# edouardlp/Mask-RCNN-CoreML

Measured on AMD Instinct MI355X. Metric: images/sec (1024x1024, COCO-80), higher is better.
Workload: dtype f32x3

## Files before the change

mask-rcnn-coreml_amd/_lib.py:

```python
from __future__ import annotations

import ctypes as C
import os

_HERE = os.path.dirname(os.path.abspath(__file__))
SO_PATH = os.environ.get("MRCNN_HIP_LIB") or os.path.join(_HERE, "libmaskrcnn_hip.so")

MRCNN_OK = 0
F32, F64, F16, U8, I32, F32S, F32X3 = 0, 1, 2, 3, 4, 5, 6
DEFAULT = -1
HOST, DEVICE = 0, 1
PARAM_INT, PARAM_DOUBLE, PARAM_STRING = 0, 1, 2
MODEL_MASKRCNN, MODEL_CLASSIFIER, MODEL_MASK = 0, 1, 2

EXPORTED_SYMBOLS = [
    "mrcnn_last_error", "mrcnn_version", "mrcnn_device_count", "mrcnn_config_set_anchors_path",
    "mrcnn_config_set_classifier_path", "mrcnn_config_set_mask_path", "mrcnn_config_get_anchors_path",
    "mrcnn_config_get_classifier_path", "mrcnn_config_get_mask_path", "mrcnn_layer_create",
    "mrcnn_layer_set_weight_data", "mrcnn_layer_output_shapes", "mrcnn_layer_evaluate", "mrcnn_layer_destroy",
    "mrcnn_iou", "mrcnn_model_load", "mrcnn_model_destroy", "mrcnn_model_set_stream", "mrcnn_maskrcnn_predict",
    "mrcnn_maskrcnn_predict_async", "mrcnn_maskrcnn_submit", "mrcnn_maskrcnn_collect", "mrcnn_classifier_predict", "mrcnn_mask_predict", "mrcnn_model_get_int",
    "mrcnn_model_read_tensor", "mrcnn_model_enable_timing", "mrcnn_model_stage_ms", "mrcnn_model_enable_graph",
    "mrcnn_detections_decode", "mrcnn_mask_to_u8", "mrcnn_paste_masks", "mrcnn_generate_anchors",
    "mrcnn_letterbox_geometry", "mrcnn_letterbox_rgb", "mrcnn_model_check_range", "mrcnn_model_calibrate_split", "mrcnn_model_split_group_stat",
# ... 10 lines not shown
    "mrcnn_jpeg_info", "mrcnn_jpeg_decode_host", "mrcnn_jpeg_decode_batch", "mrcnn_maskrcnn_predict_jpegs",
    "mrcnn_jpeg_decode_batch_on", "mrcnn_maskrcnn_predict_jpegs_on",
    "mrcnn_jpeg_encode_host", "mrcnn_jpeg_encode_batch",
    "mrcnn_png_encode_host", "mrcnn_png_encode_batch",
    "mrcnn_tile_plan", "mrcnn_maskrcnn_predict_tiles", "mrcnn_merge_tiles", "mrcnn_merge_tiles_host",
    "mrcnn_unite_tiles", "mrcnn_unite_tiles_host",
    "mrcnn_rle_decode", "mrcnn_rle_decode_host", "mrcnn_instance_map_rle", "mrcnn_instance_map_rle_host",
    "mrcnn_render_detections_rle", "mrcnn_render_detections_rle_host",
    "mrcnn_rle_to_polygons", "mrcnn_rle_to_polygons_host",
    "mrcnn_polygons_simplify", "mrcnn_polygons_simplify_host",
]
TEST_SYMBOLS = [
    "mrcnn_bench_conv", "mrcnn_bench_conv_dtype", "mrcnn_model_conv_profile_enable", "mrcnn_model_conv_profile_get",
    "mrcnn_model_conv_profile_shapes", "mrcnn_conv2d_nhwc", "mrcnn_debug_set", "mrcnn_bottleneck_nhwc", "mrcnn_bench_mfma_probe", "mrcnn_model_conv_profile_group", "mrcnn_bottleneck_first_nhwc", "mrcnn_bottleneck_stage_nhwc", "mrcnn_model_conv_profile_bytes",
    "mrcnn_jpeg_last_stage_ms", "mrcnn_jpeg_coefficients", "mrcnn_test_last_range_flag", "mrcnn_classifier_rows", "mrcnn_test_roi_align_nhwc_batch", "mrcnn_conv_chain_nhwc",
    "mrcnn_test_conv_form_nhwc",
]


class NativeLibraryMissing(RuntimeError):
    pass


class MrcnnError(RuntimeError):
    def __init__(self, code: int, msg: str):
        super().__init__(f"[mrcnn status {code}] {msg}")
        self.code = code


class Tensor(C.Structure):
    _fields_ = [("data", C.c_void_p), ("dtype", C.c_int32), ("memspace", C.c_int32),
# ... 169 lines not shown
    L.mrcnn_mask_to_u8.argtypes = [vp, C.c_int64, vp]
    L.mrcnn_mask_to_u8_f64.argtypes = [vp, C.c_int64, vp]
    ip = C.POINTER(C.c_int)
    L.mrcnn_letterbox_geometry.argtypes = [C.c_int] * 4 + [ip] * 4
    L.mrcnn_letterbox_rgb.argtypes = [vp, C.c_int, C.c_int, C.c_int, vp, C.c_int, C.c_int]
    L.mrcnn_generate_anchors.argtypes = [C.c_int, C.c_int, vp, C.c_int64, i64p]
    L.mrcnn_paste_masks.argtypes = [vp, C.c_int64, vp, C.c_int, C.c_int, C.c_int, C.c_int, C.c_float, C.c_int, vp]
    L.mrcnn_conv2d_nhwc.argtypes = [vp] + [C.c_int] * 4 + [vp] + [C.c_int] * 3 + [vp, vp, vp, C.c_int, C.c_int, vp]
    L.mrcnn_debug_set.argtypes = [cp, C.c_int]
    L.mrcnn_bench_mfma_probe.argtypes = [C.c_double, C.c_int, C.POINTER(C.c_double), C.POINTER(C.c_double)]
    L.mrcnn_bottleneck_first_nhwc.argtypes = [vp] + [C.c_int] * 4 + [vp] * 5 + [C.c_int, C.c_int, vp, vp]
    L.mrcnn_bottleneck_stage_nhwc.argtypes = [vp] + [C.c_int] * 4 + [vp] * 4 + [C.c_int, C.c_int, vp, vp, vp]
    L.mrcnn_bottleneck_nhwc.argtypes = [vp] + [C.c_int] * 4 + [vp] * 9 + [C.c_int, C.c_int, vp, vp]
    L.mrcnn_test_last_range_flag.argtypes = [ip]
    L.mrcnn_conv_chain_nhwc.argtypes = [vp] + [C.c_int] * 4 + [vp] * 5 + [C.c_int, C.c_int] + [vp] * 6 + [C.c_int] * 3 + [vp, vp]
    L.mrcnn_classifier_rows.argtypes = [vp, C.c_int64, vp, C.c_int, C.c_int64, vp, vp]
    L.mrcnn_model_check_range.argtypes = [vp, ip]
    L.mrcnn_model_calibrate_split.argtypes = [vp, vp, C.c_int, C.c_int, C.c_int, C.c_int, C.c_int]
    L.mrcnn_model_split_group_stat.argtypes = [vp, C.c_int, C.POINTER(SplitGroupStat)]
    L.mrcnn_model_get_split_exponents.argtypes = [vp, vp, C.c_int, ip]
    L.mrcnn_model_set_split_exponents.argtypes = [vp, vp, C.c_int]
    L.mrcnn_dist_rccl_shared.argtypes = []
    L.mrcnn_dist_rccl_shared.restype = C.c_int
    L.mrcnn_dist_unique_id.argtypes = [vp]
    L.mrcnn_dist_init.argtypes = [C.c_int, C.c_int, vp, C.POINTER(vp)]
    L.mrcnn_dist_destroy.argtypes = [vp]
    L.mrcnn_dist_destroy.restype = None
    L.mrcnn_dist_shard.argtypes = [C.c_int, C.c_int, C.c_int, ip, ip]
    L.mrcnn_dist_record_floats.argtypes = [C.c_int, C.c_int]
    L.mrcnn_dist_record_floats.restype = C.c_int64
# ... 39 lines not shown
```

mask-rcnn-coreml_amd/csrc/conv_dispatch.hip:

```cpp
#include "conv_device.h"
#include "knobs.h"

namespace mrcnn {

void conv_mfma_launch(hipStream_t s, const ConvArgs& a, int mode, int bn, bool wide_waves);
void conv_pp_launch(hipStream_t s, const ConvArgs& a, int mode);
void conv_chain_launch(hipStream_t s, const ConvArgs& p, const ConvArgs& q, int parts, bool wlds, int n_cus);

static inline int conv_wdtype(const ConvDesc& d) { return d.wdtype < 0 ? d.dtype : d.wdtype; }
static inline bool conv_is_split(const ConvDesc& d) { return d.dtype == MRCNN_F32 && (conv_wdtype(d) == MRCNN_F16 || conv_wdtype(d) == MRCNN_F32X3); }
static inline int conv_split_parts(const ConvDesc& d) { return conv_wdtype(d) == MRCNN_F32X3 ? 3 : 2; }
static inline bool conv_is_f16(const ConvDesc& d) { return d.dtype == MRCNN_F16 && (d.wdtype < 0 || d.wdtype == MRCNN_F16) && !d.out_f32; }
static inline bool is_pointwise(const ConvDesc& d) { return d.KH == 1 && d.KW == 1 && d.stride == 1 && !d.padH && !d.padW; }
static inline bool is_3x3_same(const ConvDesc& d) { return d.KH == 3 && d.KW == 3 && d.stride == 1 && d.padH == 1 && d.padW == 1; }
static inline bool dense_in(const ConvDesc& d, int h, int w, int c) { return d.H == h && d.W == w && d.Cin == c && d.in_sW == c && d.in_sH == (long)w * c && d.in_sB == (long)h * w * c; }
static inline bool dense_out(const ConvDesc& d, int h, int w, int c) { return d.OH == h && d.OW == w && d.Cout == c && d.out_sP == c && d.out_sB == (long)h * w * c; }
static inline bool plain_epilogue(const ConvDesc& d, int act) { return !d.out2 && !d.deconv2 && !d.sel_partial && !d.head_w && d.res_shift == 0 && d.act == act && d.scale && d.shift; }
static inline bool fills_chip(long tiles, int n_cus) { return tiles * 8 >= (long)n_cus * 7; }

static thread_local ConvProfile* g_prof = nullptr;
void conv_set_profiler(ConvProfile* p) { g_prof = p; }
static thread_local int* g_range_flag = nullptr;
void conv_set_range_flag(int* device_flag) { g_range_flag = device_flag; }
void ConvProfile::reset()
// ... 80 lines not shown
static int& g_tail = knob("conv_tail", "MRCNN_TAIL", 0);
static int& g_bneck = knob("conv_bneck", "MRCNN_BNECK", 1);
static int& g_bneck_stage = knob("conv_bneck_stage", "MRCNN_BNECK_STAGE", 0);
static int& g_c3h = knob("conv_c3h", "MRCNN_C3H", 1);
int conv_c3h_mode() { return g_c3h; }
bool conv_bneck_enabled() { return g_bneck != 0; }
static int& g_scfuse = knob("conv_scfuse", "MRCNN_SCFUSE", 1);
static int& g_sel_wave = knob("mask_sel_wave", "MRCNN_SEL_WAVE", 1);
int conv_sel_part_cols() { return g_sel_wave ? 64 : 128; }
static int& g_kchunk = knob("conv_kchunk", "MRCNN_KCHUNK", 1);
static int& g_ksplit = knob("conv_ksplit", "MRCNN_KSPLIT", 1);
static int& g_ksplit_below = knob("conv_ksplit_below", "MRCNN_KSPLIT_BELOW", 256);
static int& g_halo = knob("conv_halo", "MRCNN_HALO", 1);
bool conv_halo_enabled() { return g_halo != 0; }
static int& g_chain = knob("conv_chain", "MRCNN_CHAIN", 1);
static int& g_tn4 = knob("conv_tn4", nullptr, -1);

static int& g_pp = knob("conv_pp", "MRCNN_PP", 1);
static int& g_pp_min_tiles = knob("conv_pp_min_tiles", "MRCNN_PP_MIN_TILES", 512);
static int& g_pp_min_kt = knob("conv_pp_min_kt", "MRCNN_PP_MIN_KT", 16);
static int& g_pp_dbg = knob("conv_pp_dbg", "MRCNN_PP_DBG", 0);
static int& g_pp_min_fill = knob("conv_pp_min_fill", "MRCNN_PP_MIN_FILL", 85);
static int& g_pp_split = knob("conv_pp_split", "MRCNN_PP_SPLIT", 0);

static void conv_fill_args(const ConvDesc& d, ConvArgs& a)
{
    const bool half = d.dtype == MRCNN_F16;
    a.in = d.in; a.wgt = d.wgt; a.scale = d.scale; a.shift = d.shift; a.res = d.res; a.out = d.out; a.out2 = d.out2;
    a.in_sB = d.in_sB; a.in_sH = d.in_sH; a.in_sW = d.in_sW;
    a.res_sB = d.res_sB; a.res_sH = d.res_sH; a.res_sW = d.res_sW;
// ... 196 lines not shown
{
    if (!conv_is_split(d3) || !conv_is_split(d1) || conv_wdtype(d3) != conv_wdtype(d1)) return false;
    if (!d3.wgt_halo || !d1.wgt_halo || !conv_halo_eligible(d3) || d3.head_w || !conv_halo_tail_geometry_ok(d3.H, d3.W)) return false;
    if (d3.Npad != 256 || d3.act != ACT_RELU) return false;
    if (!conv_halo_tail_packable(d1.KH, d1.KW, d1.Cin, d1.Npad) || d1.Cout != 1024 || !is_pointwise(d1)) return false;
    if (d1.deconv2 || d1.out2 || d1.sel_partial || d1.act == ACT_SIGMOID || d1.res_shift || d1.head_w) return false;
    if (d1.in != d3.out || d1.B != d3.B || d1.OH != d3.OH || d1.OW != d3.OW) return false;
    if (!dense_out(d3, d3.OH, d3.OW, 256) || !dense_in(d1, d3.OH, d3.OW, 256)) return false;
    return true;
}

bool conv_chain_fusable(const ConvDesc& dP, const ConvDesc& dQ, const ConvDesc* sc)
{
    if (!conv_is_split(dP) || !conv_is_split(dQ) || conv_wdtype(dP) != conv_wdtype(dQ)) return false;
    const int C = dQ.Cout, H = dP.OH, W = dP.OW;
    if (!(C == 64 || C == 128) || dQ.Npad != C || dP.Cin != C || dP.Cout != 4 * C || dP.Npad != 4 * C) return false;
    if (!is_pointwise(dP) || !is_pointwise(dQ) || dP.B != dQ.B) return false;
    if (!plain_epilogue(dP, ACT_RELU) || !plain_epilogue(dQ, ACT_RELU) || dQ.res) return false;
    if (!dense_in(dP, H, W, C) || !dense_out(dP, H, W, 4 * C) || dQ.in != dP.out || !dense_in(dQ, H, W, 4 * C) || !dense_out(dQ, H, W, C)) return false;
    if (conv_k_chunks(dP) != 1 || conv_k_chunks(dQ) != 1) return false;
    auto al = [](const void* p) { return (reinterpret_cast<uintptr_t>(p) & 15) == 0; };
    if (!al(dP.in) || !al(dP.out) || !al(dQ.out) || !al(dP.wgt) || !al(dQ.wgt) || !al(dP.scale) || !al(dP.shift) || !al(dQ.scale) || !al(dQ.shift)) return false;
    if (sc) {
        if (!g_scfuse || !conv_shortcut_fusable(dP, *sc) || conv_k_chunks(*sc) != 1 || !sc->scale || !sc->shift) return false;
        if (C == 64 && sc->Cin != 64) return false;
        if (!al(sc->in) || !al(sc->wgt) || !al(sc->scale) || !al(sc->shift) || sc->in_sW % 4 || sc->in_sH % 4 || sc->in_sB % 4 || sc->Npad != 4 * C) return false;
    } else {
        if (!dP.res || !al(dP.res) || dP.res_sW != 4 * C || dP.res_sH != (long)W * 4 * C || dP.res_sB != (long)H * W * 4 * C) return false;
    }
    return true;
}

void conv_forward_chain(hipStream_t s, const ConvDesc& dP, const ConvDesc& dQ, const ConvDesc* sc)
{
    const long tiles = ((long)dP.B * dP.OH * dP.OW + 127) / 128;
    const bool sc_rides = g_chain >= 3 ? sc != nullptr && conv_chain_fusable(dP, dQ, sc) : conv_shortcut_rides(dP, sc);
    const int n_cus = device_cu_count();
    bool chain = g_chain && g_direct >= 2 && conv_chain_fusable(dP, dQ, sc_rides ? sc : nullptr) && (g_chain >= 2 || (dQ.Cout == 64 && fills_chip(tiles, n_cus)));
#ifndef MRCNN_CONV_ABLATE
    if (g_pp_dbg) chain = false;
#endif
    if (!chain) {
        conv_forward(s, dP, sc);
        conv_forward(s, dQ);
        return;
    }
    if (sc && !sc_rides) { conv_forward(s, *sc); sc = nullptr; }
    ConvDesc d = dP;
    if (sc) { d.res = nullptr; d.res_sB = d.res_sH = d.res_sW = 0; }
    ConvArgs aP, aQ;
    conv_fill_args(d, aP);
    conv_fill_args(dQ, aQ);
    if (sc) {
        aP.sc_in = sc->in; aP.sc_wgt = sc->wgt; aP.sc_scale = sc->scale; aP.sc_shift = sc->shift;
        aP.sc_in_sB = sc->in_sB; aP.sc_in_sH = sc->in_sH; aP.sc_in_sW = sc->in_sW;
        aP.sc_H = sc->H; aP.sc_W = sc->W; aP.sc_Cin = sc->Cin; aP.sc_stride = sc->stride;
    }
    const ProfScope prof(s);
    conv_chain_launch(s, aP, aQ, conv_split_parts(dP), dQ.Cout == 64, n_cus);
    if (prof) {
        const double fl = 2.0 * (double)aP.M * ((double)aP.ncols * (aP.Ktot + (sc ? sc->Cin : 0)) + (double)aQ.ncols * aQ.Ktot);
        prof.finish(sc ? TILE_128x128_4WAVE : TILE_128x128, fl, aP.M, aP.ncols, aP.Ktot, dP.group,
                    conv_algorithmic_bytes(d, sc) + conv_algorithmic_bytes(dQ) - (double)aP.M * dQ.Cin * 4.0);
    }
    HIP_CHECK(hipGetLastError());
}

void conv_forward_tail(hipStream_t s, const ConvDesc& d3, const ConvDesc& d1, const ConvDesc* sc, const ConvDesc* q)
{
    const int n_cus = device_cu_count();
    const long tiles = ((long)d3.B * d3.OH * d3.OW + 127) / 128;
    ConvArgs a3, a1;
    bool fuse = g_tail && g_halo && g_scratch && conv_tail_fusable(d3, d1) && fills_chip(tiles, n_cus);
    if (sc && fuse) { conv_forward(s, *sc); sc = nullptr; }
// ... 126 lines not shown
```

mask-rcnn-coreml_amd/csrc/conv_pack.h:

```cpp
#pragma once
#include <stddef.h>
#include <vector>

namespace mrcnn {

template <class Src>
std::vector<float> pack_filter_rows(int O, int I, int KH, int KW, int Npad, Src&& src)
{
    std::vector<float> w((size_t)Npad * KH * KW * I, 0.f);
    for (int o = 0; o < O; ++o)
        for (int y = 0; y < KH; ++y)
            for (int x = 0; x < KW; ++x)
                for (int i = 0; i < I; ++i) w[(((size_t)o * KH + y) * KW + x) * I + i] = src(o, y, x, i);
    return w;
}

inline int deconv2_row(int dy, int dx, int co, int O) { return (dy * 2 + dx) * O + co; }
template <class Src>
std::vector<float> pack_deconv2_rows(int I, int O, int Npad, Src&& src)
{
    std::vector<float> w((size_t)Npad * I, 0.f);
    for (int dy = 0; dy < 2; ++dy)
        for (int dx = 0; dx < 2; ++dx)
            for (int o = 0; o < O; ++o)
                for (int i = 0; i < I; ++i) w[(size_t)deconv2_row(dy, dx, o, O) * I + i] = src(dy, dx, o, i);
    return w;
}

}
```

mask-rcnn-coreml_amd/csrc/engine.h:

```cpp
#pragma once
#include <functional>
#include <map>
#include <mutex>
#include <memory>
#include <string>
#include <vector>

#include "kernels.h"

namespace mrcnn {

struct MrcwTensor {
    int dtype = 0;
    std::vector<uint32_t> dims;
    const unsigned char* data = nullptr;
    size_t nbytes = 0;
    size_t count() const { size_t n = 1; for (auto d : dims) n *= d; return n; }
};
struct MrcwFile {
    std::string path;
    std::vector<unsigned char> buf;
    std::map<std::string, int64_t> ints;
    std::map<std::string, double> doubles;
    std::map<std::string, std::string> strings;
// ... 4 lines not shown
    double get_double(const std::string& k, double dflt) const;
    std::string get_string(const std::string& k) const;
    const MrcwTensor& tensor(const std::string& name) const;
    std::vector<float> floats(const std::string& name) const;
};

inline int mode_act(int mode) { return (mode == MRCNN_F32S || mode == MRCNN_F32X3) ? MRCNN_F32 : mode; }
inline int mode_wgt(int mode) { return mode == MRCNN_F32 ? MRCNN_F32 : (mode == MRCNN_F32X3 ? MRCNN_F32X3 : MRCNN_F16); }

struct PackedConv {
    DevBuf wgt, scale, shift;
    std::vector<float> h_scale, h_shift;
    DevBuf wgt_halo;
    DevBuf wgt_c3h;
    DevBuf wgt_frag;
    int Cin = 0, Cout = 0, KH = 1, KW = 1, Npad = 0;
    int dtype = MRCNN_F32;
    int wdtype = MRCNN_F32;
};

struct Tensor4 {
    void* p = nullptr;
    int H = 0, W = 0, C = 0;
    long sB() const { return (long)H * W * C; }
};

using Op = std::function<void(hipStream_t, int )>;

struct SplitGroup {
    std::string name;
// ... 186 lines not shown
```

mask-rcnn-coreml_amd/csrc/engine_internal.h:

```cpp
#pragma once
#include "engine.h"

namespace mrcnn {

float half_to_float(uint16_t h);
void upload(DevBuf& d, const std::vector<float>& h);
PackedConv pack_conv_oihw(const MrcwFile& f, const std::string& conv, const std::string& bn, int mode);
PackedConv pack_conv1(const MrcwFile& f, int mode);
PackedConv pack_stacked_1x1(const MrcwFile& f, const std::vector<std::string>& names, int mode);
PackedConv pack_deconv2(const MrcwFile& f, const std::string& name, int mode);
void init_scaled_op(ScaledOp& op, const PackedConv* pc, int g_in, int g_out);

struct ConvView {
    void* p = nullptr;
    int H = 0, W = 0;
    long sB = 0, sH = 0, sW = 0;
};
inline ConvView dense_view(const void* p, int H, int W, int C)
{
    return {const_cast<void*>(p), H, W, (long)H * W * C, (long)W * C, (long)C};
}
inline ConvView view_of(const Tensor4& t) { return dense_view(t.p, t.H, t.W, t.C); }

enum : unsigned { RETILED_NONE = 0, RETILED_HALO = 1, RETILED_C3H = 2, RETILED_FRAG = 4, RETILED_ALL = 7 };

inline ConvDesc make_conv_desc(const PackedConv& pc, const float* scale, const float* shift, const ConvView& in, const ConvView& out,
                               int stride, int pad, int act, unsigned retiled)
{
    ConvDesc d;
    d.dtype = pc.dtype; d.wdtype = pc.wdtype;
    d.in = in.p; d.H = in.H; d.W = in.W; d.Cin = pc.Cin;
    d.in_sB = in.sB; d.in_sH = in.sH; d.in_sW = in.sW;
    d.wgt = pc.wgt.p; d.KH = pc.KH; d.KW = pc.KW; d.stride = stride; d.padH = d.padW = pad;
    if (retiled & RETILED_HALO) d.wgt_halo = pc.wgt_halo.p;
    if (retiled & RETILED_C3H) d.wgt_c3h = pc.wgt_c3h.p;
    if (retiled & RETILED_FRAG) d.wgt_frag = pc.wgt_frag.p;
    d.scale = scale; d.shift = shift;
    d.act = act;
    d.out = out.p; d.OH = out.H; d.OW = out.W; d.Cout = pc.Cout; d.Npad = pc.Npad;
    d.out_sB = out.sB; d.out_sP = out.sW;
    return d;
}
inline void set_residual(ConvDesc& d, const ConvView& res, int res_shift)
{
    d.res = res.p; d.res_sB = res.sB; d.res_sH = res.sH; d.res_sW = res.sW; d.res_shift = res_shift;
}

void run_conv_dense(hipStream_t s, const PackedConv& pc, const void* in, int B, int H, int W, void* out, int stride,
                    int pad, int act, const void* res = nullptr, int out_f32 = 0, const ScaledOp* sop = nullptr);

template <class F>
// ... 12 lines not shown
```

mask-rcnn-coreml_amd/csrc/engine_plan.hip:

```cpp
#include "engine_internal.h"

#include <math.h>
#include <string.h>

#include <fstream>

namespace mrcnn {

static void read_std(const MrcwFile& f, const std::string& prefix, float out[4])
{
    const float dflt[4] = {0.1f, 0.1f, 0.2f, 0.2f};
    const int64_t cnt = f.get_int(prefix + "bboxStdDev_count", 0);
    for (int i = 0; i < 4; ++i) out[i] = dflt[i];
    if (cnt == 4)
        for (int i = 0; i < 4; ++i) out[i] = (float)f.get_double(prefix + "bboxStdDev_" + std::to_string(i), dflt[i]);
}

void Model::load(int kind_, const std::string& path, int max_batch_, int dtype_)
{
    require_gpu();
    kind = kind_;
    max_batch = max_batch_ > 0 ? max_batch_ : 1;
    file.load(path);
    mode = dtype_;
// ... 299 lines not shown
        x = xo;
        g_x = g_c1;
    }

    void residual_stage(int st)
    {
        const int f1s[6] = {0, 0, 64, 128, 256, 512}, f3s[6] = {0, 0, 256, 512, 1024, 2048};
        Tensor4 stage_ta, stage_tb, stage_main, stage_alt;
        bool stage_fused = false, x_is_main = true;
        const int g_stage = m.new_split_group("C" + std::to_string(st));
        for (auto& b : blocks[st]) {
            const std::string p = std::to_string(st) + b;
            const bool first = b == "a";
            const int stride = (first && st > 2) ? 2 : 1;
            const int oh = x.H / stride, ow = x.W / stride;
            const bool chain_q = pending_tail.open && !first && (st == 2 || st == 3) && (m.mode == MRCNN_F32S || m.mode == MRCNN_F32X3);
            if (!chain_q) tail_flush();
            if (first) { stage_ta = T(oh, ow, f1s[st]); stage_tb = T(oh, ow, f1s[st]); }
            if (first && m.mode == MRCNN_F16 && blocks[st].size() > 1 && bneck_geometry_ok(f1s[st], oh, ow)) {
                stage_fused = true;
                stage_alt = T(oh, ow, f3s[st]);
            }
            const int g_a = m.new_split_group("res" + p + "_branch2a"), g_b = m.new_split_group("res" + p + "_branch2b");
            Tensor4 ta = stage_ta;
            Tensor4 tb = stage_tb;
            if (!first && stage_fused) {
                const Tensor4 to = x_is_main ? stage_alt : stage_main;
                bneck_op("res" + p + "_branch2a", "res" + p + "_branch2b", "res" + p + "_branch2c", x, ta, tb, to, g_x, g_a, g_b, g_stage);
                x = to;
                x_is_main = !x_is_main;
                g_x = g_stage;
// ... 200 lines not shown
```

mask-rcnn-coreml_amd/csrc/engine_weights.hip:

```cpp
#include "engine_internal.h"
#include "conv_pack.h"

#include <math.h>
#include <string.h>

#include <fstream>

namespace mrcnn {

float half_to_float(uint16_t h)
{
    const uint32_t sign = (uint32_t)(h & 0x8000u) << 16;
    uint32_t exp = (h >> 10) & 0x1Fu, man = h & 0x3FFu, f;
    if (exp == 0) {
        if (man == 0) f = sign;
        else {
            exp = 113;
            while ((man & 0x400u) == 0) { man <<= 1; --exp; }
            man &= 0x3FFu;
            f = sign | (exp << 23) | (man << 13);
        }
    } else if (exp == 31) f = sign | 0x7F800000u | (man << 13);
    else f = sign | ((exp + 112) << 23) | (man << 13);
    float r;
// ... 181 lines not shown
    MRCNN_REQUIRE(t.dims.size() == 4, MRCNN_ERR_IO, "%s/kernel is not 4-D", conv.c_str());
    const int O = t.dims[0], I = t.dims[1], KH = t.dims[2], KW = t.dims[3];
    const std::vector<float> k = f.floats(conv + "/kernel");
    PackedConv pc = new_pack(dtype, I, O, KH, KW);
    const std::vector<float> w = pack_filter_rows(O, I, KH, KW, pc.Npad, [&](int o, int y, int x, int i) { return k[(((size_t)o * I + i) * KH + y) * KW + x]; });
    std::vector<float> sc, sh;
    fold_bn(f, conv, bn, O, pc.Npad, sc, sh);
    finish_pack(pc, w, sc, sh);
    if (pc.wdtype != pc.dtype && conv_halo_packable(KH, KW, I, pc.Npad)) {
        conv_halo_pack(nullptr, pc.wgt.p, pc.Npad, I, pc.wgt_halo);
        HIP_CHECK(hipStreamSynchronize(nullptr));
    } else if (pc.wdtype != pc.dtype && conv_halo_tail_packable(KH, KW, I, pc.Npad) && O == pc.Npad) {
        conv_halo_pack(nullptr, pc.wgt.p, pc.Npad, I, pc.wgt_halo, 1);
        HIP_CHECK(hipStreamSynchronize(nullptr));
    }
    if (pc.dtype == MRCNN_F16 && pc.wdtype == MRCNN_F16 && conv3x3h_packable(KH, KW, I, O, pc.Npad)) {
        conv3x3h_pack(nullptr, pc.wgt.p, O, I, pc.wgt_c3h);
        HIP_CHECK(hipStreamSynchronize(nullptr));
    }
    if (pc.dtype == MRCNN_F16 && pc.wdtype == MRCNN_F16 && O == pc.Npad && bneck_frag_wanted(KH, KW, I, O)) {
        bneck_pack_frag(nullptr, pc.wgt.p, O, KH * KW * I, pc.wgt_frag);
        HIP_CHECK(hipStreamSynchronize(nullptr));
    }
    return pc;
}

PackedConv pack_conv1(const MrcwFile& f, int dtype)
{
    const MrcwTensor& t = f.tensor("conv1/kernel");
    MRCNN_REQUIRE(t.dims.size() == 4 && t.dims[1] == 3 && t.dims[2] == 7 && t.dims[3] == 7, MRCNN_ERR_IO, "conv1/kernel must be [O,3,7,7]");
// ... 68 lines not shown
```

mask-rcnn-coreml_amd/csrc/kernels.h:

```cpp
#pragma once
#include <stddef.h>
#include <algorithm>
#include <map>
#include <tuple>
#include <vector>

#include "common.h"

namespace mrcnn {


struct ProposalWorkspace {
    int B = 0, A = 0, K = 0, Kpad = 0, max_keep = 0, nblk = 0, W = 0;
    uint32_t* keys = nullptr;
    uint32_t* hist = nullptr;
    uint32_t* blockhist = nullptr;
    uint32_t* state = nullptr;
    uint64_t* cand = nullptr;
    int32_t* topk_idx = nullptr;
    float* boxes = nullptr;
    uint64_t* nms_mask = nullptr;
    int32_t* keep_idx = nullptr;
    int32_t* keep_count = nullptr;
    static size_t bytes(int B, int A, int K, int max_keep);
// ... 138 lines not shown
void png_encode_forward(hipStream_t s, const PngBuffers& b, int batch, long long total_blocks, int format, int rows);

enum Act { ACT_NONE = 0, ACT_RELU = 1, ACT_SIGMOID = 2 };

struct ConvDesc {
    int dtype = MRCNN_F32;
    int out_f32 = 0;
    int wdtype = -1;
    const void* in = nullptr;
    int B = 0, H = 0, W = 0, Cin = 0;
    long in_sB = 0, in_sH = 0, in_sW = 0;
    const void* wgt = nullptr;
    const void* wgt_halo = nullptr;
    const void* wgt_frag = nullptr;
    const void* wgt_c3h = nullptr;
    int prefer_c3h = 0;
    int KH = 1, KW = 1, stride = 1, padH = 0, padW = 0;
    const float* scale = nullptr;
    const float* shift = nullptr;
    const void* res = nullptr;
    long res_sB = 0, res_sH = 0, res_sW = 0;
    int res_shift = 0;
    int act = ACT_NONE;
    void* out = nullptr;
    int OH = 0, OW = 0, Cout = 0, Npad = 0;
    long out_sB = 0, out_sP = 0;
    void* out2 = nullptr;
    int n_split = 0;
    long out2_sB = 0, out2_sP = 0;
    int deconv2 = 0;
// ... 223 lines not shown
```

mask-rcnn-coreml_amd/csrc/kernels_conv_chain.hip:

```cpp
#include "conv_device.h"

namespace mrcnn {

struct ChainArgs { ConvArgs p, q; };

__device__ __forceinline__ void chain_stage_acc(float* stage, const f32x16& acc, int l31, int kk)
{
#pragma unroll
    for (int q = 0; q < 4; ++q)
        *reinterpret_cast<float4*>(&stage[l31 * 32 + (((2 * q + kk) ^ (l31 & 7)) << 2)]) = make_float4(acc[4 * q], acc[4 * q + 1], acc[4 * q + 2], acc[4 * q + 3]);
}

struct ChainParts { f16x8 hi, lo, lo2; };
template <int PARTS>
__device__ __forceinline__ ChainParts chain_split(const uint4 u0, const uint4 u1)
{
    ChainParts p;
    if constexpr (PARTS == 3) split_hi_mid_lo(u0, u1, p.hi, p.lo, p.lo2);
    else { split_hi_lo(u0, u1, p.hi, p.lo); p.lo2 = p.lo; }
    return p;
}
template <int PARTS, int N>
__device__ __forceinline__ void chain_mfma_parts(f32x16 (&acc)[N], const uint4 (&bv)[N], const ChainParts& pt)
{
    const f16x8 hi = pt.hi, lo = pt.lo, lo2 = pt.lo2;
    _Pragma("unroll") for (int j = 0; j < N; ++j) acc[j] = __builtin_amdgcn_mfma_f32_32x32x16_f16(__builtin_bit_cast(f16x8, bv[j]), hi, acc[j], 0, 0, 0);
    _Pragma("unroll") for (int j = 0; j < N; ++j) acc[j] = __builtin_amdgcn_mfma_f32_32x32x16_f16(__builtin_bit_cast(f16x8, bv[j]), lo, acc[j], 0, 0, 0);
    if constexpr (PARTS == 3)
        _Pragma("unroll") for (int j = 0; j < N; ++j) acc[j] = __builtin_amdgcn_mfma_f32_32x32x16_f16(__builtin_bit_cast(f16x8, bv[j]), lo2, acc[j], 0, 0, 0);
}

template <int C, int PARTS, bool SC, bool WLDS>
__global__ __launch_bounds__(WLDS ? 512 : 256, WLDS ? 1 : 2) void k_conv_chain(const ChainArgs ca)
{
    static_assert(!WLDS || C == 64, "the LDS-resident form holds C = 64's filters");
    constexpr int NW = WLDS ? 8 : 4, C4 = 4 * C, KT = C / 32, TNP = 2, TNQ = C / 32;
    constexpr int A_BYTES = WLDS ? 0 : KT * 32 * 128;
    constexpr int W_BYTES = WLDS ? C4 * C * 2 : 0;
    constexpr int WF_BYTES = W_BYTES * (SC ? 3 : 2);
    __shared__ __attribute__((aligned(16))) unsigned char smem[WF_BYTES + NW * (A_BYTES + 32 * 32 * 4)];
    const ConvArgs& a = ca.p;
    const ConvArgs& aq = ca.q;
    const int t = threadIdx.x;
    const int wave = t >> 6, lane = t & 63;
// ... 195 lines not shown
            float4 x = *reinterpret_cast<const float4*>(&stage[(8 * ps + rrow) * 32 + (((lane & 7) ^ rrow) << 2)]);
            x.x = x.x * sc.x + sh.x; x.y = x.y * sc.y + sh.y; x.z = x.z * sc.z + sh.z; x.w = x.w * sc.w + sh.w;
            if (reluq) { x.x = fmaxf(x.x, 0.f); x.y = fmaxf(x.y, 0.f); x.z = fmaxf(x.z, 0.f); x.w = fmaxf(x.w, 0.f); }
            if (ok[ps]) {
                out_of_range_q = out_of_range_q || !(fabsf(x.x) < 65504.0f) || !(fabsf(x.y) < 65504.0f) || !(fabsf(x.z) < 65504.0f) || !(fabsf(x.w) < 65504.0f);
                *reinterpret_cast<float4*>(outq + mrow[ps] * C + n) = x;
            }
        }
        __builtin_amdgcn_wave_barrier();
    }
    }
    if (a.range_flag && out_of_range) atomicOr(a.range_flag, 1);
    if (aq.range_flag && out_of_range_q) atomicOr(aq.range_flag, 1);
}

void conv_chain_launch(hipStream_t s, const ConvArgs& p, const ConvArgs& q, int parts, bool wlds, int n_cus)
{
    ChainArgs ca{p, q};
    dim3 grid((p.M + 127) / 128), block(256);
    const bool sc = p.sc_in != nullptr;
    const int C = q.Cout;
    MRCNN_REQUIRE((C == 64 || C == 128) && (parts == 2 || parts == 3), MRCNN_ERR_INVALID, "conv_chain_launch: C %d, %d parts", C, parts);
    if (wlds) {
        MRCNN_REQUIRE(C == 64 && (!sc || p.sc_Cin == 64) && n_cus > 0, MRCNN_ERR_INVALID, "conv_chain_launch: the LDS-resident form holds C = 64's filters");
        const int tiles256 = (p.M + 255) / 256;
        grid = dim3(tiles256 < n_cus ? tiles256 : n_cus); block = dim3(512);
#define MRCNN_CHAIN_W(P_, S_) hipLaunchKernelGGL((k_conv_chain<64, P_, S_, true>), grid, block, 0, s, ca)
        if (parts == 3) { if (sc) MRCNN_CHAIN_W(3, true); else MRCNN_CHAIN_W(3, false); }
        else { if (sc) MRCNN_CHAIN_W(2, true); else MRCNN_CHAIN_W(2, false); }
#undef MRCNN_CHAIN_W
        return;
    }
    MRCNN_REQUIRE(C == 128, MRCNN_ERR_INVALID, "conv_chain_launch: C = 64 runs the LDS-resident form");
#define MRCNN_CHAIN(C_, P_, S_) hipLaunchKernelGGL((k_conv_chain<C_, P_, S_, false>), grid, block, 0, s, ca)
    if (parts == 3) { if (sc) MRCNN_CHAIN(128, 3, true); else MRCNN_CHAIN(128, 3, false); }
    else { if (sc) MRCNN_CHAIN(128, 2, true); else MRCNN_CHAIN(128, 2, false); }
#undef MRCNN_CHAIN
// ... 4 lines not shown
```

Before: 457.0.

## Extend fused 1x1 conv chain to C=256 stage-4 pairs with LDS weight ring

Adds a new chain kernel for ResNet stage-4 identity blocks (C=256, 1024 expand). The expand conv's output is fed straight into the following reduce conv inside one kernel, so the intermediate activation is not written and re-read between launches. The fp16 filter chunks are prepacked into a swizzled stream image at load time and double-buffered into LDS with buffer_load ... lds DMA. This costs extra weight memory and one large-LDS block per CU, and it relies on hand-written inline asm and waitcnt counts.

```diff
diff --git a/mask-rcnn-coreml_amd/_lib.py b/mask-rcnn-coreml_amd/_lib.py
--- a/mask-rcnn-coreml_amd/_lib.py
+++ b/mask-rcnn-coreml_amd/_lib.py
@@ -48,7 +48,7 @@
     "mrcnn_bench_conv", "mrcnn_bench_conv_dtype", "mrcnn_model_conv_profile_enable", "mrcnn_model_conv_profile_get",
     "mrcnn_model_conv_profile_shapes", "mrcnn_conv2d_nhwc", "mrcnn_debug_set", "mrcnn_bottleneck_nhwc", "mrcnn_bench_mfma_probe", "mrcnn_model_conv_profile_group", "mrcnn_bottleneck_first_nhwc", "mrcnn_bottleneck_stage_nhwc", "mrcnn_model_conv_profile_bytes",
     "mrcnn_jpeg_last_stage_ms", "mrcnn_jpeg_coefficients", "mrcnn_test_last_range_flag", "mrcnn_classifier_rows", "mrcnn_test_roi_align_nhwc_batch", "mrcnn_conv_chain_nhwc",
-    "mrcnn_test_conv_form_nhwc",
+    "mrcnn_test_conv_form_nhwc", "mrcnn_test_chain_stream_image",
 ]
 
 
@@ -248,6 +248,7 @@
     L.mrcnn_bottleneck_nhwc.argtypes = [vp] + [C.c_int] * 4 + [vp] * 9 + [C.c_int, C.c_int, vp, vp]
     L.mrcnn_test_last_range_flag.argtypes = [ip]
     L.mrcnn_conv_chain_nhwc.argtypes = [vp] + [C.c_int] * 4 + [vp] * 5 + [C.c_int, C.c_int] + [vp] * 6 + [C.c_int] * 3 + [vp, vp]
+    L.mrcnn_test_chain_stream_image.argtypes = [vp, C.c_int, C.c_int, vp]
     L.mrcnn_classifier_rows.argtypes = [vp, C.c_int64, vp, C.c_int, C.c_int64, vp, vp]
     L.mrcnn_model_check_range.argtypes = [vp, ip]
     L.mrcnn_model_calibrate_split.argtypes = [vp, vp, C.c_int, C.c_int, C.c_int, C.c_int, C.c_int]
diff --git a/mask-rcnn-coreml_amd/csrc/conv_dispatch.hip b/mask-rcnn-coreml_amd/csrc/conv_dispatch.hip
--- a/mask-rcnn-coreml_amd/csrc/conv_dispatch.hip
+++ b/mask-rcnn-coreml_amd/csrc/conv_dispatch.hip
@@ -5,7 +5,7 @@
 
 void conv_mfma_launch(hipStream_t s, const ConvArgs& a, int mode, int bn, bool wide_waves);
 void conv_pp_launch(hipStream_t s, const ConvArgs& a, int mode);
-void conv_chain_launch(hipStream_t s, const ConvArgs& p, const ConvArgs& q, int parts, bool wlds, int n_cus);
+void conv_chain_launch(hipStream_t s, const ConvArgs& p, const ConvArgs& q, int parts, bool wlds, int n_cus, const void* p_stream, const void* q_stream);
 
 static inline int conv_wdtype(const ConvDesc& d) { return d.wdtype < 0 ? d.dtype : d.wdtype; }
 static inline bool conv_is_split(const ConvDesc& d) { return d.dtype == MRCNN_F32 && (conv_wdtype(d) == MRCNN_F16 || conv_wdtype(d) == MRCNN_F32X3); }
@@ -118,6 +118,7 @@
 static int& g_halo = knob("conv_halo", "MRCNN_HALO", 1);
 bool conv_halo_enabled() { return g_halo != 0; }
 static int& g_chain = knob("conv_chain", "MRCNN_CHAIN", 1);
+static int& g_chain4 = knob("conv_chain4", "MRCNN_CHAIN4", 1);
 static int& g_tn4 = knob("conv_tn4", nullptr, -1);
 
 static int& g_pp = knob("conv_pp", "MRCNN_PP", 1);
@@ -344,13 +345,14 @@
 {
     if (!conv_is_split(dP) || !conv_is_split(dQ) || conv_wdtype(dP) != conv_wdtype(dQ)) return false;
     const int C = dQ.Cout, H = dP.OH, W = dP.OW;
-    if (!(C == 64 || C == 128) || dQ.Npad != C || dP.Cin != C || dP.Cout != 4 * C || dP.Npad != 4 * C) return false;
+    if (!(C == 64 || C == 128 || C == 256) || dQ.Npad != C || dP.Cin != C || dP.Cout != 4 * C || dP.Npad != 4 * C) return false;
     if (!is_pointwise(dP) || !is_pointwise(dQ) || dP.B != dQ.B) return false;
     if (!plain_epilogue(dP, ACT_RELU) || !plain_epilogue(dQ, ACT_RELU) || dQ.res) return false;
     if (!dense_in(dP, H, W, C) || !dense_out(dP, H, W, 4 * C) || dQ.in != dP.out || !dense_in(dQ, H, W, 4 * C) || !dense_out(dQ, H, W, C)) return false;
     if (conv_k_chunks(dP) != 1 || conv_k_chunks(dQ) != 1) return false;
     auto al = [](const void* p) { return (reinterpret_cast<uintptr_t>(p) & 15) == 0; };
     if (!al(dP.in) || !al(dP.out) || !al(dQ.out) || !al(dP.wgt) || !al(dQ.wgt) || !al(dP.scale) || !al(dP.shift) || !al(dQ.scale) || !al(dQ.shift)) return false;
+    if (C == 256 && (sc || !dP.wgt_stream || !dQ.wgt_stream || !al(dP.wgt_stream) || !al(dQ.wgt_stream))) return false;
     if (sc) {
         if (!g_scfuse || !conv_shortcut_fusable(dP, *sc) || conv_k_chunks(*sc) != 1 || !sc->scale || !sc->shift) return false;
         if (C == 64 && sc->Cin != 64) return false;
@@ -366,7 +368,9 @@
     const long tiles = ((long)dP.B * dP.OH * dP.OW + 127) / 128;
     const bool sc_rides = g_chain >= 3 ? sc != nullptr && conv_chain_fusable(dP, dQ, sc) : conv_shortcut_rides(dP, sc);
     const int n_cus = device_cu_count();
-    bool chain = g_chain && g_direct >= 2 && conv_chain_fusable(dP, dQ, sc_rides ? sc : nullptr) && (g_chain >= 2 || (dQ.Cout == 64 && fills_chip(tiles, n_cus)));
+    const bool c4 = dQ.Cout == 256;
+    const int g = c4 ? g_chain4 : g_chain;
+    bool chain = g && g_direct >= 2 && !(c4 && sc) && conv_chain_fusable(dP, dQ, sc_rides ? sc : nullptr) && (g >= 2 || ((c4 || dQ.Cout == 64) && fills_chip(tiles, n_cus)));
 #ifndef MRCNN_CONV_ABLATE
     if (g_pp_dbg) chain = false;
 #endif
@@ -387,7 +391,7 @@
         aP.sc_H = sc->H; aP.sc_W = sc->W; aP.sc_Cin = sc->Cin; aP.sc_stride = sc->stride;
     }
     const ProfScope prof(s);
-    conv_chain_launch(s, aP, aQ, conv_split_parts(dP), dQ.Cout == 64, n_cus);
+    conv_chain_launch(s, aP, aQ, conv_split_parts(dP), dQ.Cout == 64, n_cus, dP.wgt_stream, dQ.wgt_stream);
     if (prof) {
         const double fl = 2.0 * (double)aP.M * ((double)aP.ncols * (aP.Ktot + (sc ? sc->Cin : 0)) + (double)aQ.ncols * aQ.Ktot);
         prof.finish(sc ? TILE_128x128_4WAVE : TILE_128x128, fl, aP.M, aP.ncols, aP.Ktot, dP.group,
diff --git a/mask-rcnn-coreml_amd/csrc/conv_pack.h b/mask-rcnn-coreml_amd/csrc/conv_pack.h
--- a/mask-rcnn-coreml_amd/csrc/conv_pack.h
+++ b/mask-rcnn-coreml_amd/csrc/conv_pack.h
@@ -27,4 +27,25 @@
     return w;
 }
 
+inline bool chain_stream_wanted(int KH, int KW, int I, int O) { return KH == 1 && KW == 1 && ((I == 256 && O == 1024) || (I == 1024 && O == 256)); }
+inline size_t chain_stream_pos_p(int C, int n, int k)
+{
+    const int r = n & 63;
+    return (size_t)(n >> 6) * 64 * C + ((size_t)(k >> 5) * 64 + r) * 32 + ((((k >> 3) & 3) ^ ((r >> 2) & 3)) << 3) + (k & 7);
 }
+inline size_t chain_stream_pos_q(int C, int n, int k)
+{
+    return (size_t)(k >> 6) * 64 * C + ((size_t)((k >> 5) & 1) * C + n) * 32 + ((((k >> 3) & 3) ^ ((n >> 2) & 3)) << 3) + (k & 7);
+}
+template <class T>
+std::vector<T> pack_chain_stream(const T* w, int C, bool q)
+{
+    static_assert(sizeof(T) == 2, "fp16 filters");
+    const int rows = q ? C : 4 * C, K = q ? 4 * C : C;
+    std::vector<T> img((size_t)rows * K);
+    for (int n = 0; n < rows; ++n)
+        for (int k = 0; k < K; ++k) img[q ? chain_stream_pos_q(C, n, k) : chain_stream_pos_p(C, n, k)] = w[(size_t)n * K + k];
+    return img;
+}
+
+}
diff --git a/mask-rcnn-coreml_amd/csrc/engine.h b/mask-rcnn-coreml_amd/csrc/engine.h
--- a/mask-rcnn-coreml_amd/csrc/engine.h
+++ b/mask-rcnn-coreml_amd/csrc/engine.h
@@ -42,6 +42,7 @@
     DevBuf wgt_halo;
     DevBuf wgt_c3h;
     DevBuf wgt_frag;
+    DevBuf wgt_stream;
     int Cin = 0, Cout = 0, KH = 1, KW = 1, Npad = 0;
     int dtype = MRCNN_F32;
     int wdtype = MRCNN_F32;
diff --git a/mask-rcnn-coreml_amd/csrc/engine_internal.h b/mask-rcnn-coreml_amd/csrc/engine_internal.h
--- a/mask-rcnn-coreml_amd/csrc/engine_internal.h
+++ b/mask-rcnn-coreml_amd/csrc/engine_internal.h
@@ -22,7 +22,7 @@
 }
 inline ConvView view_of(const Tensor4& t) { return dense_view(t.p, t.H, t.W, t.C); }
 
-enum : unsigned { RETILED_NONE = 0, RETILED_HALO = 1, RETILED_C3H = 2, RETILED_FRAG = 4, RETILED_ALL = 7 };
+enum : unsigned { RETILED_NONE = 0, RETILED_HALO = 1, RETILED_C3H = 2, RETILED_FRAG = 4, RETILED_STREAM = 8, RETILED_ALL = 15 };
 
 inline ConvDesc make_conv_desc(const PackedConv& pc, const float* scale, const float* shift, const ConvView& in, const ConvView& out,
                                int stride, int pad, int act, unsigned retiled)
@@ -35,6 +35,7 @@
     if (retiled & RETILED_HALO) d.wgt_halo = pc.wgt_halo.p;
     if (retiled & RETILED_C3H) d.wgt_c3h = pc.wgt_c3h.p;
     if (retiled & RETILED_FRAG) d.wgt_frag = pc.wgt_frag.p;
+    if (retiled & RETILED_STREAM) d.wgt_stream = pc.wgt_stream.p;
     d.scale = scale; d.shift = shift;
     d.act = act;
     d.out = out.p; d.OH = out.H; d.OW = out.W; d.Cout = pc.Cout; d.Npad = pc.Npad;
diff --git a/mask-rcnn-coreml_amd/csrc/engine_plan.hip b/mask-rcnn-coreml_amd/csrc/engine_plan.hip
--- a/mask-rcnn-coreml_amd/csrc/engine_plan.hip
+++ b/mask-rcnn-coreml_amd/csrc/engine_plan.hip
@@ -337,7 +337,7 @@
             const bool first = b == "a";
             const int stride = (first && st > 2) ? 2 : 1;
             const int oh = x.H / stride, ow = x.W / stride;
-            const bool chain_q = pending_tail.open && !first && (st == 2 || st == 3) && (m.mode == MRCNN_F32S || m.mode == MRCNN_F32X3);
+            const bool chain_q = pending_tail.open && !first && (st == 2 || st == 3 || (st == 4 && !pending_tail.has_sc)) && (m.mode == MRCNN_F32S || m.mode == MRCNN_F32X3);
             if (!chain_q) tail_flush();
             if (first) { stage_ta = T(oh, ow, f1s[st]); stage_tb = T(oh, ow, f1s[st]); }
             if (first && m.mode == MRCNN_F16 && blocks[st].size() > 1 && bneck_geometry_ok(f1s[st], oh, ow)) {
diff --git a/mask-rcnn-coreml_amd/csrc/engine_weights.hip b/mask-rcnn-coreml_amd/csrc/engine_weights.hip
--- a/mask-rcnn-coreml_amd/csrc/engine_weights.hip
+++ b/mask-rcnn-coreml_amd/csrc/engine_weights.hip
@@ -219,6 +219,13 @@
         conv_halo_pack(nullptr, pc.wgt.p, pc.Npad, I, pc.wgt_halo, 1);
         HIP_CHECK(hipStreamSynchronize(nullptr));
     }
+    if (pc.wdtype != pc.dtype && pc.dtype == MRCNN_F32 && O == pc.Npad && chain_stream_wanted(KH, KW, I, O) && conv.find("_branch2") != std::string::npos) {
+        std::vector<uint16_t> hw(w.size());
+        for (size_t i = 0; i < w.size(); ++i) hw[i] = float_to_half(w[i]);
+        const std::vector<uint16_t> img = pack_chain_stream(hw.data(), 256, I == 1024);
+        pc.wgt_stream.alloc(img.size() * 2);
+        HIP_CHECK(hipMemcpy(pc.wgt_stream.p, img.data(), img.size() * 2, hipMemcpyHostToDevice));
+    }
     if (pc.dtype == MRCNN_F16 && pc.wdtype == MRCNN_F16 && conv3x3h_packable(KH, KW, I, O, pc.Npad)) {
         conv3x3h_pack(nullptr, pc.wgt.p, O, I, pc.wgt_c3h);
         HIP_CHECK(hipStreamSynchronize(nullptr));
diff --git a/mask-rcnn-coreml_amd/csrc/kernels.h b/mask-rcnn-coreml_amd/csrc/kernels.h
--- a/mask-rcnn-coreml_amd/csrc/kernels.h
+++ b/mask-rcnn-coreml_amd/csrc/kernels.h
@@ -176,6 +176,7 @@
     const void* wgt_halo = nullptr;
     const void* wgt_frag = nullptr;
     const void* wgt_c3h = nullptr;
+    const void* wgt_stream = nullptr;
     int prefer_c3h = 0;
     int KH = 1, KW = 1, stride = 1, padH = 0, padW = 0;
     const float* scale = nullptr;
diff --git a/mask-rcnn-coreml_amd/csrc/kernels_conv_chain.hip b/mask-rcnn-coreml_amd/csrc/kernels_conv_chain.hip
--- a/mask-rcnn-coreml_amd/csrc/kernels_conv_chain.hip
+++ b/mask-rcnn-coreml_amd/csrc/kernels_conv_chain.hip
@@ -2,7 +2,7 @@
 
 namespace mrcnn {
 
-struct ChainArgs { ConvArgs p, q; };
+struct ChainArgs { ConvArgs p, q; const void *p_stream, *q_stream; };
 
 __device__ __forceinline__ void chain_stage_acc(float* stage, const f32x16& acc, int l31, int kk)
 {
@@ -20,14 +20,14 @@
     else { split_hi_lo(u0, u1, p.hi, p.lo); p.lo2 = p.lo; }
     return p;
 }
-template <int PARTS, int N>
-__device__ __forceinline__ void chain_mfma_parts(f32x16 (&acc)[N], const uint4 (&bv)[N], const ChainParts& pt)
+template <int PARTS, int N, int NA = N, int OFF = 0>
+__device__ __forceinline__ void chain_mfma_parts(f32x16 (&acc)[NA], const uint4 (&bv)[N], const ChainParts& pt)
 {
     const f16x8 hi = pt.hi, lo = pt.lo, lo2 = pt.lo2;
-    _Pragma("unroll") for (int j = 0; j < N; ++j) acc[j] = __builtin_amdgcn_mfma_f32_32x32x16_f16(__builtin_bit_cast(f16x8, bv[j]), hi, acc[j], 0, 0, 0);
-    _Pragma("unroll") for (int j = 0; j < N; ++j) acc[j] = __builtin_amdgcn_mfma_f32_32x32x16_f16(__builtin_bit_cast(f16x8, bv[j]), lo, acc[j], 0, 0, 0);
+    _Pragma("unroll") for (int j = 0; j < N; ++j) acc[OFF + j] = __builtin_amdgcn_mfma_f32_32x32x16_f16(__builtin_bit_cast(f16x8, bv[j]), hi, acc[OFF + j], 0, 0, 0);
+    _Pragma("unroll") for (int j = 0; j < N; ++j) acc[OFF + j] = __builtin_amdgcn_mfma_f32_32x32x16_f16(__builtin_bit_cast(f16x8, bv[j]), lo, acc[OFF + j], 0, 0, 0);
     if constexpr (PARTS == 3)
-        _Pragma("unroll") for (int j = 0; j < N; ++j) acc[j] = __builtin_amdgcn_mfma_f32_32x32x16_f16(__builtin_bit_cast(f16x8, bv[j]), lo2, acc[j], 0, 0, 0);
+        _Pragma("unroll") for (int j = 0; j < N; ++j) acc[OFF + j] = __builtin_amdgcn_mfma_f32_32x32x16_f16(__builtin_bit_cast(f16x8, bv[j]), lo2, acc[OFF + j], 0, 0, 0);
 }
 
 template <int C, int PARTS, bool SC, bool WLDS>
@@ -253,13 +253,224 @@
     if (aq.range_flag && out_of_range_q) atomicOr(aq.range_flag, 1);
 }
 
-void conv_chain_launch(hipStream_t s, const ConvArgs& p, const ConvArgs& q, int parts, bool wlds, int n_cus)
-{
-    ChainArgs ca{p, q};
+template <int C, int PARTS>
+__global__ __launch_bounds__(256, 1) void k_conv_chain_ring(const ChainArgs ca)
+{
+    static_assert(C == 256, "the ring's stage holds C = 256's chunk images");
+    constexpr int C4 = 4 * C, KT = C / 32, TNP = 2, TNQ = C / 32, NCH = C4 / 64;
+    constexpr int WCH = 64 * C * 2;
+    constexpr int STAGE = 2 * WCH;
+    constexpr int NDMA = WCH / 4096;
+    __shared__ __attribute__((aligned(16))) unsigned char smem[2 * STAGE + 4 * 32 * 32 * 4];
+    __shared__ __attribute__((aligned(16))) float s_tab[2 * C4], s_tabq[2 * C];
+    const ConvArgs& a = ca.p;
+    const ConvArgs& aq = ca.q;
+    const int t = threadIdx.x;
+    const int wave = t >> 6, lane = t & 63;
+    const int l31 = lane & 31, kk = lane >> 5;
+    float* const stage = reinterpret_cast<float*>(smem + 2 * STAGE) + wave * (32 * 32);
+    static_assert(C4 == 4 * 256 && C % 8 == 0 && C / 2 <= 256, "the tables are filled by 256 threads, 16 B each");
+    *reinterpret_cast<float4*>(&s_tab[4 * t]) = *reinterpret_cast<const float4*>(a.scale + 4 * t);
+    *reinterpret_cast<float4*>(&s_tab[C4 + 4 * t]) = *reinterpret_cast<const float4*>(a.shift + 4 * t);
+    if (t < C / 2) *reinterpret_cast<float4*>(&s_tabq[4 * t]) = *reinterpret_cast<const float4*>(t < C / 4 ? aq.scale + 4 * t : aq.shift + 4 * (t - C / 4));
+    const float* const in = static_cast<const float*>(a.in);
+    const float* const res = static_cast<const float*>(a.res);
+    float* const out = static_cast<float*>(a.out);
+    float* const outq = static_cast<float*>(aq.out);
+    const int swzb = (l31 >> 2) & 3;
+
+    typedef unsigned srd_t __attribute__((ext_vector_type(4)));
+    srd_t srdP, srdQ;
+    {
+        const unsigned long long wp = (unsigned long long)(uintptr_t)ca.p_stream, wq = (unsigned long long)(uintptr_t)ca.q_stream;
+        srdP[0] = __builtin_amdgcn_readfirstlane((unsigned)wp);
+        srdP[1] = __builtin_amdgcn_readfirstlane((unsigned)(wp >> 32) & 0xffffu);
+        srdP[2] = (unsigned)(NCH * WCH);
+        srdP[3] = 0x00020000u;
+        srdQ[0] = __builtin_amdgcn_readfirstlane((unsigned)wq);
+        srdQ[1] = __builtin_amdgcn_readfirstlane((unsigned)(wq >> 32) & 0xffffu);
+        srdQ[2] = (unsigned)(NCH * WCH);
+        srdQ[3] = 0x00020000u;
+    }
+    const unsigned lds0 = __builtin_amdgcn_readfirstlane((unsigned)(uintptr_t)(__attribute__((address_space(3))) unsigned char*)smem);
+    const unsigned wdst = lds0 + (unsigned)__builtin_amdgcn_readfirstlane(wave) * 1024u;
+    const unsigned voff = (unsigned)t * 16u;
+#define MRCNN_RING_DMA(SRD, SOFF, DST)                                                                         \
+    asm volatile("s_nop 4\n\ts_mov_b32 m0, %3\n\ts_nop 0\n\tbuffer_load_dwordx4 %0, %1, %2 offen lds" ::"v"(voff), "s"(SRD), "s"(SOFF), "s"(DST) : "memory", "m0");
+    auto ring_fill = [&](int ch) {
+        const unsigned src = (unsigned)__builtin_amdgcn_readfirstlane(ch) * (unsigned)WCH;
+        const unsigned dst = wdst + (unsigned)(__builtin_amdgcn_readfirstlane(ch) & 1) * (unsigned)STAGE;
+#pragma unroll
+        for (int k = 0; k < NDMA; ++k) {
+            MRCNN_RING_DMA(srdP, src + k * 4096u, dst + k * 4096u)
+            MRCNN_RING_DMA(srdQ, src + k * 4096u, dst + (unsigned)WCH + k * 4096u)
+        }
+    };
+    ring_fill(0);
+
+    const int row0 = (blockIdx.x * 4 + __builtin_amdgcn_readfirstlane(wave)) * 32;
+    const bool live = row0 < a.M;
+    bool out_of_range = false, out_of_range_q = false;
+    ChainParts ap[2 * KT];
+    if (live) {
+        const int m = row0 + l31;
+        const bool m_ok = m < a.M;
+        const float* const src = in + (long)(m_ok ? m : row0) * C + 8 * kk;
+        uint4 u[2 * KT][2];
+#pragma unroll
+        for (int g = 0; g < 2 * KT; ++g) { u[g][0] = *reinterpret_cast<const uint4*>(src + g * 16); u[g][1] = *reinterpret_cast<const uint4*>(src + g * 16 + 4); }
+#pragma unroll
+        for (int g = 0; g < 2 * KT; ++g) {
+            if (!m_ok) u[g][0] = u[g][1] = make_uint4(0u, 0u, 0u, 0u);
+            ap[g] = chain_split<PARTS>(u[g][0], u[g][1]);
+        }
+    }
+    const bool full = row0 + 32 <= a.M;
+    const int rrow = lane >> 3, c4 = (lane & 7) * 4;
+    const bool relu = a.act == ACT_RELU, reluq = aq.act == ACT_RELU;
+    bool ok[4];
+    long mrow[4];
+#pragma unroll
+    for (int ps = 0; ps < 4; ++ps) { const int m = row0 + 8 * ps + rrow; ok[ps] = m < a.M; mrow[ps] = m; }
+
+    f32x16 accQ[TNQ];
+#pragma unroll
+    for (int j = 0; j < TNQ; ++j)
+#pragma unroll
+        for (int e = 0; e < 16; ++e) accQ[j][e] = 0.0f;
+
+    for (int ch = 0; ch < NCH; ++ch) {
+        if (full) asm volatile("s_waitcnt vmcnt(4)" ::: "memory");
+        else asm volatile("s_waitcnt vmcnt(0)" ::: "memory");
+        __syncthreads();
+        if (ch + 1 < NCH) ring_fill(ch + 1);
+        if (!live) continue;
+        const unsigned char* const w3s = smem + (ch & 1) * STAGE;
+        const unsigned char* const w1s = w3s + WCH;
+        const int nc = ch * 64;
+        float4 rv[TNP][4];
+#pragma unroll
+        for (int j = 0; j < TNP; ++j)
+#pragma unroll
+            for (int ps = 0; ps < 4; ++ps) {
+                rv[j][ps] = make_float4(0.f, 0.f, 0.f, 0.f);
+                if (res && ok[ps]) rv[j][ps] = *reinterpret_cast<const float4*>(res + mrow[ps] * C4 + nc + j * 32 + c4);
+            }
+        f32x16 accP[TNP];
+#pragma unroll
+        for (int j = 0; j < TNP; ++j)
+#pragma unroll
+            for (int e = 0; e < 16; ++e) accP[j][e] = 0.0f;
+        auto frag_p = [&](uint4 (&b)[TNP], int i) {
+#pragma unroll
+            for (int j = 0; j < TNP; ++j) b[j] = *reinterpret_cast<const uint4*>(w3s + ((i >> 1) * 64 + j * 32 + l31) * 64 + (((2 * (i & 1) + kk) ^ swzb) << 4));
+        };
+        {
+            uint4 bv[TNP];
+            frag_p(bv, 0);
+#pragma unroll
+            for (int i = 0; i < 2 * KT; ++i) {
+                uint4 bn[TNP];
+                if (i + 1 < 2 * KT) frag_p(bn, i + 1);
+                __builtin_amdgcn_sched_barrier(0);
+                chain_mfma_parts<PARTS, TNP>(accP, bv, ap[i]);
+                if (i + 1 < 2 * KT) {
+#pragma unroll
+                    for (int j = 0; j < TNP; ++j) bv[j] = bn[j];
+                }
+            }
+        }
+        auto frag_q = [&](uint4 (&b)[TNQ / 2], int j, int h) {
+#pragma unroll
+            for (int i = 0; i < TNQ / 2; ++i) b[i] = *reinterpret_cast<const uint4*>(w1s + (j * C + ((h & 1) * (TNQ / 2) + i) * 32 + l31) * 64 + (((2 * (h >> 1) + kk) ^ swzb) << 4));
+        };
+#pragma unroll
+        for (int j = 0; j < TNP; ++j) {
+            const int n = nc + j * 32 + c4;
+            uint4 bq[TNQ / 2];
+            frag_q(bq, j, 0);
+            chain_stage_acc(stage, accP[j], l31, kk);
+            __builtin_amdgcn_wave_barrier();
+            const float4 sc = *reinterpret_cast<const float4*>(&s_tab[n]), sh = *reinterpret_cast<const float4*>(&s_tab[C4 + n]);
+            float4 xs[4];
+#pragma unroll
+            for (int ps = 0; ps < 4; ++ps) xs[ps] = *reinterpret_cast<const float4*>(&stage[(8 * ps + rrow) * 32 + (((lane & 7) ^ rrow) << 2)]);
+#pragma unroll
+            for (int ps = 0; ps < 4; ++ps) {
+                float4 x = xs[ps];
+                x.x = x.x * sc.x + sh.x; x.y = x.y * sc.y + sh.y; x.z = x.z * sc.z + sh.z; x.w = x.w * sc.w + sh.w;
+                if (res) { x.x += rv[j][ps].x; x.y += rv[j][ps].y; x.z += rv[j][ps].z; x.w += rv[j][ps].w; }
+                if (relu) { x.x = fmaxf(x.x, 0.f); x.y = fmaxf(x.y, 0.f); x.z = fmaxf(x.z, 0.f); x.w = fmaxf(x.w, 0.f); }
+                if (ok[ps]) {
+                    out_of_range = out_of_range || !(fabsf(x.x) < 65504.0f) || !(fabsf(x.y) < 65504.0f) || !(fabsf(x.z) < 65504.0f) || !(fabsf(x.w) < 65504.0f);
+                    *reinterpret_cast<float4*>(out + mrow[ps] * C4 + n) = x;
+                }
+                xs[ps] = x;
+            }
+            __builtin_amdgcn_wave_barrier();
+#pragma unroll
+            for (int ps = 0; ps < 4; ++ps) *reinterpret_cast<float4*>(&stage[(8 * ps + rrow) * 32 + (((lane & 7) ^ rrow) << 2)]) = xs[ps];
+            __builtin_amdgcn_wave_barrier();
+            ChainParts pt;
+#pragma unroll
+            for (int h = 0; h < 4; ++h) {
+                if ((h & 1) == 0) {
+                    const int g = h >> 1;
+                    const uint4 u0 = *reinterpret_cast<const uint4*>(&stage[l31 * 32 + (((4 * g + 2 * kk) ^ (l31 & 7)) << 2)]);
+                    const uint4 u1 = *reinterpret_cast<const uint4*>(&stage[l31 * 32 + (((4 * g + 2 * kk + 1) ^ (l31 & 7)) << 2)]);
+                    pt = chain_split<PARTS>(u0, u1);
+                }
+                uint4 bn[TNQ / 2];
+                if (h < 3) frag_q(bn, j, h + 1);
+                __builtin_amdgcn_sched_barrier(0);
+                if (h & 1) chain_mfma_parts<PARTS, TNQ / 2, TNQ, TNQ / 2>(accQ, bq, pt);
+                else chain_mfma_parts<PARTS, TNQ / 2, TNQ, 0>(accQ, bq, pt);
+                if (h < 3) {
+#pragma unroll
+                    for (int i = 0; i < TNQ / 2; ++i) bq[i] = bn[i];
+                }
+            }
+            __builtin_amdgcn_wave_barrier();
+        }
+    }
+#undef MRCNN_RING_DMA
+    if (live) {
+#pragma unroll
+        for (int jq = 0; jq < TNQ; ++jq) {
+            const int n = jq * 32 + c4;
+            chain_stage_acc(stage, accQ[jq], l31, kk);
+            __builtin_amdgcn_wave_barrier();
+            const float4 sc = *reinterpret_cast<const float4*>(&s_tabq[n]), sh = *reinterpret_cast<const float4*>(&s_tabq[C + n]);
+#pragma unroll
+            for (int ps = 0; ps < 4; ++ps) {
+                float4 x = *reinterpret_cast<const float4*>(&stage[(8 * ps + rrow) * 32 + (((lane & 7) ^ rrow) << 2)]);
+                x.x = x.x * sc.x + sh.x; x.y = x.y * sc.y + sh.y; x.z = x.z * sc.z + sh.z; x.w = x.w * sc.w + sh.w;
+                if (reluq) { x.x = fmaxf(x.x, 0.f); x.y = fmaxf(x.y, 0.f); x.z = fmaxf(x.z, 0.f); x.w = fmaxf(x.w, 0.f); }
+                if (ok[ps]) {
+                    out_of_range_q = out_of_range_q || !(fabsf(x.x) < 65504.0f) || !(fabsf(x.y) < 65504.0f) || !(fabsf(x.z) < 65504.0f) || !(fabsf(x.w) < 65504.0f);
+                    *reinterpret_cast<float4*>(outq + mrow[ps] * C + n) = x;
+                }
+            }
+            __builtin_amdgcn_wave_barrier();
+        }
+    }
+    if (a.range_flag && out_of_range) atomicOr(a.range_flag, 1);
+    if (aq.range_flag && out_of_range_q) atomicOr(aq.range_flag, 1);
+}
+
+void conv_chain_launch(hipStream_t s, const ConvArgs& p, const ConvArgs& q, int parts, bool wlds, int n_cus, const void* p_stream, const void* q_stream)
+{
+    ChainArgs ca{p, q, p_stream, q_stream};
     dim3 grid((p.M + 127) / 128), block(256);
     const bool sc = p.sc_in != nullptr;
     const int C = q.Cout;
-    MRCNN_REQUIRE((C == 64 || C == 128) && (parts == 2 || parts == 3), MRCNN_ERR_INVALID, "conv_chain_launch: C %d, %d parts", C, parts);
+    MRCNN_REQUIRE((C == 64 || C == 128 || C == 256) && (parts == 2 || parts == 3), MRCNN_ERR_INVALID, "conv_chain_launch: C %d, %d parts", C, parts);
+    if (C == 256) {
+        MRCNN_REQUIRE(!wlds && !sc && p.res && p_stream && q_stream, MRCNN_ERR_INVALID, "conv_chain_launch: C = 256 runs identity pairs from their stream images");
+        if (parts == 3) hipLaunchKernelGGL((k_conv_chain_ring<256, 3>), grid, block, 0, s, ca);
+        else hipLaunchKernelGGL((k_conv_chain_ring<256, 2>), grid, block, 0, s, ca);
+        return;
+    }
     if (wlds) {
         MRCNN_REQUIRE(C == 64 && (!sc || p.sc_Cin == 64) && n_cus > 0, MRCNN_ERR_INVALID, "conv_chain_launch: the LDS-resident form holds C = 64's filters");
         const int tiles256 = (p.M + 255) / 256;
```

Result: faster. 463.3, median of 6 (+1.4%).
